# fhausmann/deepgrp

Hardware: AMD Instinct MI355X
Metric: Mbp/sec predicted (whole node) at window=200 stride=50, 5-class (higher is better)
Workload: dtype f16

## Files before the change

### deepgrp_amd/csrc/gru_shared.h

```cpp
#pragma once
#include "dgrp_model.h"

typedef _Float16 half8 __attribute__((ext_vector_type(8)));
typedef float f32x16 __attribute__((ext_vector_type(16)));
typedef float f32x4 __attribute__((ext_vector_type(4)));
typedef _Float16 half4 __attribute__((ext_vector_type(4)));

#define DGRP_WG_WINDOWS 16

struct gru_rec {
    int64_t idx_off, n, out_row, nwin;
    dgrp_placement place;
    int64_t win_first;
    int64_t pad_;
};

struct gru_params {
    const uint8_t *idx;
    int64_t n, s, w0, nw;
    dgrp_placement place;
    const uint4 *pack;
    const float *ffb;
    float *out;
    void *avg;
    int avg_f32;
    int T, C, nfrag, mode;
    int Tp;
    int ospan;
    const struct gru_rec *recs;
    const int64_t *wg_first;
    int64_t nrec;
    int64_t avgw;
    const uint4 *pack_lo;
    int lo_tile_off;
    float zfold;
    const uint4 *pack16;
    const float *xtab;
    int xtab_off;
    const uint4 *stream;
    const uint4 *packw;
    const float *xtabw;
    int avg_up;
};

__device__ __forceinline__ float sigmoid_from_scaled(float a) { return __builtin_amdgcn_rcpf(1.0f + __builtin_amdgcn_exp2f(a)); }
__device__ __forceinline__ float tanh_from_scaled(float a) { return 1.0f - 2.0f * __builtin_amdgcn_rcpf(1.0f + __builtin_amdgcn_exp2f(a)); }
typedef float f32x2 __attribute__((ext_vector_type(2)));
__device__ __forceinline__ f32x2 rcp1p_exp2_pair(float a0, float a1)
{
    f32x2 e = { __builtin_amdgcn_exp2f(a0), __builtin_amdgcn_exp2f(a1) };
    e = e + 1.0f;
    return f32x2{ __builtin_amdgcn_rcpf(e.x), __builtin_amdgcn_rcpf(e.y) };
}
__device__ __forceinline__ float fast_tanh(float x) { return tanh_from_scaled(2.8853900817779268f * x); }

template <int N>
__device__ __forceinline__ float row_ror(float x)
{
    return __builtin_bit_cast(float, __builtin_amdgcn_update_dpp(0, __builtin_bit_cast(int, x), 0x120 | N, 0xf, 0xf, false));
}
template <int N>
__device__ __forceinline__ float row_max_ror(float x)
{
    float r;
    asm("s_nop 1\n\tv_max_f32_dpp %0, %1, %1 row_ror:%2 row_mask:0xf bank_mask:0xf" : "=v"(r) : "v"(x), "n"(N));
    return r;
}
template <int CTRL>
__device__ __forceinline__ float quad_perm(float x)
{
    return __builtin_bit_cast(float, __builtin_amdgcn_update_dpp(0, __builtin_bit_cast(int, x), CTRL, 0xf, 0xf, false));
}
__device__ __forceinline__ float row_allmax(float x)
{
    return row_max_ror<1>(row_max_ror<2>(row_max_ror<4>(row_max_ror<8>(x))));
}
__device__ __forceinline__ float row_allsum(float x)
{
    x += row_ror<8>(x); x += row_ror<4>(x); x += row_ror<2>(x); return x + row_ror<1>(x);
}

typedef __attribute__((address_space(3))) unsigned lds_u32;
typedef __attribute__((address_space(1))) unsigned glb_u32;
__device__ __forceinline__ void lds_atomic_max(unsigned *p, unsigned v)
{
    (void)__hip_atomic_fetch_max((lds_u32 *)p, v, __ATOMIC_RELAXED, __HIP_MEMORY_SCOPE_WORKGROUP);
}
__device__ __forceinline__ void global_atomic_max(unsigned *p, unsigned v)
{
    (void)__hip_atomic_fetch_max((glb_u32 *)p, v, __ATOMIC_RELAXED, __HIP_MEMORY_SCOPE_AGENT);
}

__host__ __device__ static inline int gru_lds_hbuf(int UP, int pad = 8) { return 2 * 32 * (UP + pad) * 2; }
__host__ __device__ static inline int gru_lds_dpart(int NW) { return 2 * NW * 64 * 16; }
__host__ __device__ static inline int gru_lds_seq(int Tp) { return DGRP_WG_WINDOWS * Tp; }
__host__ __device__ static inline int gru_lds_meta() { return DGRP_WG_WINDOWS * 8 + DGRP_WG_WINDOWS * 4; }

struct wg_ctx {
    _Float16 *hbuf;
    float *dpart;
    uint8_t *seqs;
    int64_t *row0s;
    int *rowoff;
    unsigned *obuf;
    int64_t wg_w, lo;
    int nvalid;
};

template <int MODE>
__device__ __forceinline__ int64_t wg_record_at(const gru_params &pin, gru_params &p, int64_t g)
{
    if (MODE == 1 || !pin.recs) return g;
    int64_t lo_r = 0, hi_r = pin.nrec;
    while (hi_r - lo_r > 1) {
        const int64_t mid = (lo_r + hi_r) >> 1;
        if (pin.wg_first[mid] <= g) lo_r = mid; else hi_r = mid;
    }
    const gru_rec rc = pin.recs[lo_r];
    p.idx = pin.idx + rc.idx_off;
    p.n = rc.n;
    if (MODE == 0) p.out = pin.out + rc.out_row * pin.C;
    p.place = rc.place;
    p.w0 = 0;
    p.nw = rc.nwin;
    p.avgw = rc.win_first;
    return g - pin.wg_first[lo_r];
}
template <int MODE>
__device__ __forceinline__ int64_t wg_record(const gru_params &pin, gru_params &p) { return wg_record_at<MODE>(pin, p, blockIdx.x); }

template <int NW, int MODE, int HPAD = 8>
__device__ __forceinline__ wg_ctx wg_setup(const gru_params &p, unsigned char *smem, int64_t bid)
{
    constexpr int UP = 32 * NW, HS = UP + HPAD;
    wg_ctx c;
    c.hbuf = reinterpret_cast<_Float16 *>(smem);
    c.dpart = reinterpret_cast<float *>(smem + gru_lds_hbuf(UP, HPAD));
    c.seqs = smem + gru_lds_hbuf(UP, HPAD) + gru_lds_dpart(NW);
    c.row0s = reinterpret_cast<int64_t *>(c.seqs + gru_lds_seq(p.Tp));
    c.rowoff = reinterpret_cast<int *>(c.row0s + DGRP_WG_WINDOWS);
    c.obuf = reinterpret_cast<unsigned *>(c.rowoff + DGRP_WG_WINDOWS);
    const int tid = threadIdx.x, T = p.T, C = p.C;
    c.wg_w = p.w0 + bid * DGRP_WG_WINDOWS;
    c.nvalid = (int)min((int64_t)DGRP_WG_WINDOWS, p.w0 + p.nw - c.wg_w);
    for (int i = tid; i < DGRP_WG_WINDOWS * T; i += 64 * NW) {
        const int wi = i / T, t = i - wi * T;
        c.seqs[wi * p.Tp + t] = wi < c.nvalid ? p.idx[(c.wg_w + wi) * p.s + t] : (uint8_t)4;
    }
    for (int i = tid; i < 32 * HS; i += 64 * NW) c.hbuf[i] = (_Float16)0.0f;
    c.lo = 0;
    if (MODE == 0) {
        const int64_t a = dgrp_place_row(p.place, c.wg_w, p.s), b = dgrp_place_row(p.place, c.wg_w + c.nvalid - 1, p.s);
        c.lo = a < b ? a : b;
        for (int i = tid; i < p.ospan * C; i += 64 * NW) c.obuf[i] = 0u;
    }
    if (tid < DGRP_WG_WINDOWS) {
        int64_t r0 = -1;
        int off = -1;
        if (tid < c.nvalid) {
            r0 = MODE == 0 ? dgrp_place_row(p.place, c.wg_w + tid, p.s) : (c.wg_w + tid - p.w0 + p.avgw) * (int64_t)T;
            if (MODE == 0 && r0 >= c.lo && r0 - c.lo + T <= p.ospan) off = (int)(r0 - c.lo);
        }
        c.row0s[tid] = r0;
        c.rowoff[tid] = off;
    }
    __syncthreads();
    return c;
}

template <int MODE>
__device__ __forceinline__ void emit_value(const gru_params &p, const wg_ctx &c, int off, int64_t row0, int t, int cls, float val)
{
    if (MODE == 0) {
        if (off >= 0) {
            lds_atomic_max(c.obuf + (off + t) * p.C + cls, __float_as_uint(val));
        } else {
            const int64_t row = row0 + t;
            if (row < p.n) global_atomic_max(reinterpret_cast<unsigned *>(p.out) + row * p.C + cls, __float_as_uint(val));
        }
    } else {
        p.out[(row0 + t) * p.C + cls] = val;
    }
}

template <int NW, int MODE>
__device__ __forceinline__ void finish_register(const gru_params &p, const wg_ctx &c, int t, int reg, float fbias, int off, int64_t row0)
{
    const int lane = threadIdx.x & 63, cls = lane & 15;
    const float *dp = c.dpart + ((size_t)(t & 1) * 4 + reg) * NW * 64 + lane;
    float sum = dp[0];
#pragma unroll
    for (int w = 1; w < NW; ++w) sum += dp[w * 64];
    const int wi = 4 * (lane >> 4) + reg;
    const float lg = cls < p.C ? sum + fbias : -INFINITY;
    float val = lg;
    if (MODE != 2) {
        const float m = row_allmax(lg);
        const float e = __builtin_amdgcn_exp2f(1.4426950408889634f * (lg - m));
        val = e * __builtin_amdgcn_rcpf(row_allsum(e));
    }
    if (cls < p.C && wi < c.nvalid) emit_value<MODE>(p, c, off, row0, t, cls, val);
}

template <int NW>
__device__ __forceinline__ void flush_image(const gru_params &p, const wg_ctx &c)
{
    __syncthreads();
    unsigned *gout = reinterpret_cast<unsigned *>(p.out) + c.lo * p.C;
    const int64_t lim = (p.n - c.lo) * p.C;
    for (int i = threadIdx.x; i < p.ospan * p.C; i += 64 * NW) {
        const unsigned v = c.obuf[i];
        if (v != 0u && i < lim) global_atomic_max(gout + i, v);
    }
}

__device__ __forceinline__ void split_avg_store_lane(const gru_params &p, int64_t wg_w, int tt, int UP, int wave, int lane, half8 a0, half8 a1,
                                                     half8 l0, half8 l1)
{
    const int64_t at = ((wg_w + (lane & 15) - p.w0 + p.avgw) * (int64_t)p.T + tt) * UP + 32 * wave + 8 * (lane >> 4);
    if (p.avg_f32) {
        float *dst = reinterpret_cast<float *>(p.avg) + at;
        typedef unsigned u32x4_ __attribute__((ext_vector_type(4)));
        const _Float16 hf = (_Float16)0.5f;
        const u32x4_ A0 = __builtin_bit_cast(u32x4_, a0), A1 = __builtin_bit_cast(u32x4_, a1);
        const u32x4_ L0 = __builtin_bit_cast(u32x4_, l0 * hf), L1 = __builtin_bit_cast(u32x4_, l1 * hf);
        float v[8];
#pragma unroll
        for (int k = 0; k < 4; ++k) {
            float f0, f1, r0, r1;
            asm("v_fma_mix_f32 %0, %1, 0.5, %2 op_sel_hi:[1,0,1]" : "=v"(f0) : "v"(A0[k]), "v"(L0[k]));
            asm("v_fma_mix_f32 %0, %1, 0.5, %2 op_sel:[1,0,1] op_sel_hi:[1,0,1]" : "=v"(f1) : "v"(A0[k]), "v"(L0[k]));
            asm("v_fma_mix_f32 %0, %1, 0.5, %2 op_sel_hi:[1,0,1]" : "=v"(r0) : "v"(A1[k]), "v"(L1[k]));
            asm("v_fma_mix_f32 %0, %1, 0.5, %2 op_sel:[1,0,1] op_sel_hi:[1,0,1]" : "=v"(r1) : "v"(A1[k]), "v"(L1[k]));
            v[2 * k] = f0 + r0;
            v[2 * k + 1] = f1 + r1;
        }
        *reinterpret_cast<f32x4 *>(dst) = f32x4{ v[0], v[1], v[2], v[3] };
        *reinterpret_cast<f32x4 *>(dst + 4) = f32x4{ v[4], v[5], v[6], v[7] };
        return;
    }
    const _Float16 hf = (_Float16)0.5f;
    const half8 av = (a0 * hf + a1 * hf) + (l0 + l1) * hf;
    *reinterpret_cast<half8 *>(reinterpret_cast<_Float16 *>(p.avg) + at) = av;
}
__device__ __forceinline__ void split_avg_store(const gru_params &p, int64_t wg_w, int tt, int UP, int wave, half8 a0, half8 a1,
                                                half8 l0, half8 l1)
{
    split_avg_store_lane(p, wg_w, tt, UP, wave, threadIdx.x & 63, a0, a1, l0, l1);
}

struct split_gate_tmp { float er, e2, g, A, zt, d, n; };
template <bool ONERCP, int OP>
__device__ __forceinline__ void split_gate_op(split_gate_tmp &t, float ar, float ag, float az, float ax, float &s)
{
#pragma clang fp contract(off)
    if constexpr (OP == 0) t.er = __builtin_amdgcn_exp2f(ar);
    else if constexpr (OP == 1) t.e2 = __builtin_amdgcn_exp2f(az);
    else if constexpr (OP == 2) t.er = t.er + 1.0f;
    else if constexpr (OP == 3) t.er = __builtin_amdgcn_rcpf(t.er);
    else if constexpr (OP == 4) t.g = __builtin_fmaf(t.er, ag, ax);
    else if constexpr (OP == 5) t.A = __builtin_amdgcn_exp2f(t.g);
    else if constexpr (OP == 6) t.A = t.A + 1.0f;
    else if constexpr (ONERCP) {
        if constexpr (OP == 7) t.zt = __builtin_fmaf(0.5f, t.e2, 1.0f);
        else if constexpr (OP == 8) t.d = t.A * t.zt;
        else if constexpr (OP == 9) t.n = __builtin_fmaf(s, t.A, -t.e2);
        else if constexpr (OP == 10) t.d = __builtin_amdgcn_rcpf(t.d);
        else s = t.n * t.d;
    } else {
        if constexpr (OP == 7) t.zt = t.e2 + 1.0f;
        else if constexpr (OP == 8) t.d = __builtin_amdgcn_rcpf(t.A);
        else if constexpr (OP == 9) t.n = __builtin_fmaf(-2.0f, t.d, 1.0f);
        else if constexpr (OP == 10) t.zt = __builtin_amdgcn_rcpf(t.zt);
        else { const float df = s - t.n; s = __builtin_fmaf(t.zt, df, t.n); }
    }
}
#define DGRP_SPLIT_GATE_OPS 12
template <bool ONERCP>
__device__ __forceinline__ float split_gate_chain(float ar, float ag, float az, float ax, float s)
{
    split_gate_tmp t;
    split_gate_op<ONERCP, 0>(t, ar, ag, az, ax, s); split_gate_op<ONERCP, 1>(t, ar, ag, az, ax, s);
    split_gate_op<ONERCP, 2>(t, ar, ag, az, ax, s); split_gate_op<ONERCP, 3>(t, ar, ag, az, ax, s);
    split_gate_op<ONERCP, 4>(t, ar, ag, az, ax, s); split_gate_op<ONERCP, 5>(t, ar, ag, az, ax, s);
    split_gate_op<ONERCP, 6>(t, ar, ag, az, ax, s); split_gate_op<ONERCP, 7>(t, ar, ag, az, ax, s);
    split_gate_op<ONERCP, 8>(t, ar, ag, az, ax, s); split_gate_op<ONERCP, 9>(t, ar, ag, az, ax, s);
    split_gate_op<ONERCP, 10>(t, ar, ag, az, ax, s); split_gate_op<ONERCP, 11>(t, ar, ag, az, ax, s);
    return s;
}
template <bool ONERCP> __device__ __forceinline__ float split_state_h(float s)
{
#pragma clang fp contract(off)
    return ONERCP ? s + 1.0f : s;
}
__device__ __forceinline__ uint2 split_pack4(const float h[4])
{
    uint2 r;
    asm("v_cvt_pk_f16_f32 %0, %1, %2" : "=v"(r.x) : "v"(h[0]), "v"(h[1]));
    asm("v_cvt_pk_f16_f32 %0, %1, %2" : "=v"(r.y) : "v"(h[2]), "v"(h[3]));
    return r;
}
__device__ __forceinline__ void split_residual4(float h[4], uint2 hi)
{
    asm("v_fma_mix_f32 %0, %1, -1.0, %0 op_sel_hi:[1,0,0]" : "+v"(h[0]) : "v"(hi.x));
    asm("v_fma_mix_f32 %0, %1, -1.0, %0 op_sel:[1,0,0] op_sel_hi:[1,0,0]" : "+v"(h[1]) : "v"(hi.x));
    asm("v_fma_mix_f32 %0, %1, -1.0, %0 op_sel_hi:[1,0,0]" : "+v"(h[2]) : "v"(hi.y));
    asm("v_fma_mix_f32 %0, %1, -1.0, %0 op_sel:[1,0,0] op_sel_hi:[1,0,0]" : "+v"(h[3]) : "v"(hi.y));
}
__device__ __forceinline__ void split_hi_lo4(const float h[4], uint2 &hv, uint2 &lv)
{
    float r[4] = { h[0], h[1], h[2], h[3] };
    hv = split_pack4(r);
    split_residual4(r, hv);
    lv = split_pack4(r);
}

__device__ __forceinline__ float wave_half_sum(float h, float half)
{
#pragma clang fp contract(off)
    float t = half * h;
    asm("s_nop 1\n\tv_fmac_f32_dpp %0, %1, %2 row_ror:8 row_mask:0xf bank_mask:0xf" : "+v"(t) : "v"(h), "v"(half));
    return t;
}

__device__ __forceinline__ void split_lstm_cell(float ai, float af, float ac, float ao, float &c, float &h)
{
#pragma clang fp contract(off)
    const float ig = __builtin_amdgcn_rcpf(1.0f + __builtin_amdgcn_exp2f(ai));
    const float fg = __builtin_amdgcn_rcpf(1.0f + __builtin_amdgcn_exp2f(af));
    const float tc = __builtin_fmaf(-2.0f, __builtin_amdgcn_rcpf(1.0f + __builtin_amdgcn_exp2f(ac)), 1.0f);
    const float it = ig * tc;
    c = __builtin_fmaf(fg, c, it);
    const float og = __builtin_amdgcn_rcpf(1.0f + __builtin_amdgcn_exp2f(ao));
    const float e2 = __builtin_amdgcn_exp2f(2.8853900817779268f * c);
    const float th = __builtin_fmaf(-2.0f, __builtin_amdgcn_rcpf(1.0f + e2), 1.0f);
    h = og * th;
}
```

### deepgrp_amd/csrc/gru_split2.hip

```cpp
#include "gru_shared.h"
#include <mutex>
#include <type_traits>

typedef unsigned u32x4 __attribute__((ext_vector_type(4)));

namespace {

constexpr int NW = 4, UP = 128, KS = 4, HPAD = 16, HS = UP + HPAD;
constexpr int XT_PITCH = 4 * 128 * 4 + 32;

struct split2_weights {
    u32x4 hi[3][KS][2], lo[3][KS][2];
    u32x4 Bd_hi, Bd_lo;
};

#define LOAD2(a, pa, b, pb)                                                                                             \
    asm volatile("global_load_dwordx4 %0, %2, off\n\tglobal_load_dwordx4 %1, %3, off\n\ts_waitcnt vmcnt(0)"            \
                 : "=&a"(a), "=&a"(b) : "v"(pa), "v"(pb) : "memory")

#define MFMA_R(acc, Wf, b) asm volatile("v_mfma_f32_16x16x32_f16 %0, %1, %2, %0" : "+v"(acc) : "a"(Wf), "v"(b))
#define MFMA_D(acc, a, Wf) asm volatile("v_mfma_f32_16x16x32_f16 %0, %1, %2, %0" : "+v"(acc) : "v"(a), "a"(Wf))
#define MFMA_DZ(acc, a, Wf) asm volatile("v_mfma_f32_16x16x32_f16 %0, %1, %2, 0" : "=&v"(acc) : "v"(a), "a"(Wf))

struct tile_state {
    gru_params p;
    wg_ctx ctx;
    unsigned hcur, hnxt, lcur, lnxt;
    unsigned myseq;
    float h[16];
    f32x4 ar[4], ag[4], az[4], ax[4];
    f32x4 dpl;
    unsigned tabf, tabr;
    half8 f0h[2], f0l[2];
    int p_off;
    int64_t p_row0;
    bool pr_on;
};

template <int MODE, bool ONERCP>
__global__ void __launch_bounds__(256) __attribute__((amdgpu_waves_per_eu(1, 1))) gru_split2_kernel(const gru_params pin, int half_bytes)
{
    extern __shared__ __attribute__((aligned(16))) unsigned char smem[];
    const int tid = threadIdx.x;
    const int lane = tid & 63;
    const int wave = __builtin_amdgcn_readfirstlane(tid >> 6);
    const int T = pin.T, C = pin.C;

    split2_weights W;
    {
        const uint4 *p16 = pin.pack16 + (size_t)wave * 48 * 64 + lane;
#pragma unroll
        for (int g = 0; g < 3; ++g)
#pragma unroll
            for (int ks = 0; ks < KS; ++ks) {
                LOAD2(W.hi[g][ks][0], p16 + (size_t)(g * 8 + ks * 2) * 64, W.hi[g][ks][1], p16 + (size_t)(g * 8 + ks * 2 + 1) * 64);
                LOAD2(W.lo[g][ks][0], p16 + (size_t)(24 + g * 8 + ks * 2) * 64, W.lo[g][ks][1], p16 + (size_t)(24 + g * 8 + ks * 2 + 1) * 64);
            }
        const uint4 *mypack = pin.pack + (size_t)wave * pin.nfrag * 64 + lane;
        LOAD2(W.Bd_hi, mypack + (size_t)(3 * (2 * KS + 1) + 1) * 64, W.Bd_lo, mypack + (size_t)(3 * (2 * KS + 1) + 2) * 64);
    }
    for (int i = tid; i < 5 * 512; i += 256)
        *reinterpret_cast<float *>(smem + pin.xtab_off + (i / 512) * XT_PITCH + (i % 512) * 4) = pin.xtab[i];

    const int wi = lane & 15, q4 = lane >> 4;
    const int cls = lane & 15;
    const float fbias = cls < C ? pin.ffb[cls] : 0.0f;
    const int pwi = 4 * (lane >> 4) + wave;
    const unsigned frag_lane = (unsigned)(wi * HS + 8 * q4) * 2;
    const unsigned dense_lane = (unsigned)(wi * HS + 32 * wave + 8 * q4) * 2;
    const unsigned pub_lane = (unsigned)(wi * HS + 32 * wave + 4 * q4) * 2;
    const unsigned tab_lane = (unsigned)pin.xtab_off + (unsigned)(32 * wave + 4 * q4) * 4;

    tile_state S0, S1;
    auto setup = [&](tile_state &Z, int x) {
        unsigned char *base = smem + (size_t)x * half_bytes;
        _Float16 *lbuf = reinterpret_cast<_Float16 *>(base + pin.lo_tile_off);
        for (int i = tid; i < 32 * HS; i += 256) lbuf[i] = (_Float16)0.0f;
        Z.p = pin;
        const int64_t bid = wg_record_at<MODE>(pin, Z.p, 2 * (int64_t)blockIdx.x + x);
        Z.ctx = wg_setup<NW, MODE, HPAD>(Z.p, base, bid);
        Z.hcur = (unsigned)x * half_bytes;
        Z.hnxt = Z.hcur + 32 * HS * 2;
        Z.lcur = (unsigned)x * half_bytes + pin.lo_tile_off;
        Z.lnxt = Z.lcur + 32 * HS * 2;
        Z.myseq = (unsigned)(Z.ctx.seqs - smem) + wi * pin.Tp;
#pragma unroll
        for (int i = 0; i < 16; ++i) Z.h[i] = ONERCP ? -1.0f : 0.0f;
        Z.p_off = Z.ctx.rowoff[pwi];
        Z.p_row0 = Z.ctx.row0s[pwi];
        Z.pr_on = cls < C && pwi < Z.ctx.nvalid;
    };
    setup(S0, 0);
    setup(S1, 1);

    auto lds16 = [&](unsigned off) -> half8 { return *reinterpret_cast<const half8 *>(smem + off); };
    auto ldsf4 = [&](unsigned off) -> f32x4 { return *reinterpret_cast<const f32x4 *>(smem + off); };
    auto tab_rows = [&](tile_state &Z, uint32_t bf, uint32_t br) {
        bf = bf < 4 ? bf : 4;
        br = br < 4 ? 3 - br : 4;
        Z.tabf = tab_lane + bf * XT_PITCH;
        Z.tabr = tab_lane + br * XT_PITCH;
    };
    auto acc_init = [&](tile_state &Z, int g, int sub) {
        const f32x4 v = ldsf4(((sub & 1) ? Z.tabr : Z.tabf) + g * 512 + (sub >> 1) * 64);
        if (g == 0) Z.ar[sub] = v; else if (g == 1) Z.ag[sub] = v; else Z.az[sub] = v;
    };

    struct frag_ring { half8 h[2][2], l[2][2]; };
    struct dense_ops { half8 a0, a1, l0, l1; };
    struct fin_state { float d[NW], lg, m, e, s; };
    auto phase = [&](auto do_x, auto do_y, auto do_f, tile_state &X, tile_state &Y, int tx, int ty) __attribute__((always_inline)) {
        constexpr bool DO_X = decltype(do_x)::value, DO_Y = decltype(do_y)::value, DO_F = decltype(do_f)::value;
        frag_ring F;
        dense_ops D;
        fin_state fs;
        split_gate_tmp gt[16];
        float pbh[4][4];
        uint2 pbhv[4], pblv[4];
        uint32_t xp_bf = 4, xp_br = 4;
        const int td = ty - 1;
        const int tf = tx - 2;
        if constexpr (DO_X) { F.h[0][0] = X.f0h[0]; F.h[0][1] = X.f0h[1]; F.l[0][0] = X.f0l[0]; F.l[0][1] = X.f0l[1]; }
#define GAP __builtin_amdgcn_sched_barrier(0);
#define M_K(ks, n)                                                                                               \
    if constexpr (DO_X) {                                                                                        \
        constexpr int ps_ = (n) / 12, g_ = ((n) % 12) / 4, uh_ = ((n) % 4) / 2, rh_ = (n) % 2, sub_ = 2 * uh_ + rh_; \
        const half8 &b_ = ps_ == 1 ? F.l[(ks) & 1][rh_] : F.h[(ks) & 1][rh_];                                    \
        const u32x4 &w_ = ps_ == 2 ? W.lo[g_][ks][uh_] : W.hi[g_][ks][uh_];                                      \
        if constexpr (g_ == 0) MFMA_R(X.ar[sub_], w_, b_);                                                       \
        else if constexpr (g_ == 1) MFMA_R(X.ag[sub_], w_, b_);                                                  \
        else MFMA_R(X.az[sub_], w_, b_);                                                                         \
    }
#define M_D(i)                                                                                                   \
    if constexpr (DO_X) {                                                                                        \
        if constexpr ((i) == 0) MFMA_DZ(X.dpl, D.a0, W.Bd_hi);                                                   \
        else if constexpr ((i) == 1) MFMA_D(X.dpl, D.a1, W.Bd_hi);                                               \
        else if constexpr ((i) == 2) MFMA_D(X.dpl, D.a0, W.Bd_lo);                                               \
        else if constexpr ((i) == 3) MFMA_D(X.dpl, D.a1, W.Bd_lo);                                               \
        else if constexpr ((i) == 4) MFMA_D(X.dpl, D.l0, W.Bd_hi);                                               \
        else MFMA_D(X.dpl, D.l1, W.Bd_hi);                                                                       \
    }
#define PF(ks)                                                                                                   \
    if constexpr (DO_X) {                                                                                        \
        F.h[(ks) & 1][0] = lds16(X.hcur + frag_lane + 64 * (ks)); F.h[(ks) & 1][1] = lds16(X.hcur + frag_lane + 16 * HS * 2 + 64 * (ks)); \
        F.l[(ks) & 1][0] = lds16(X.lcur + frag_lane + 64 * (ks)); F.l[(ks) & 1][1] = lds16(X.lcur + frag_lane + 16 * HS * 2 + 64 * (ks)); \
    }
#define RDD                                                                                                      \
    if constexpr (DO_X) {                                                                                        \
        D.a0 = lds16(X.hcur + dense_lane); D.a1 = lds16(X.hcur + dense_lane + 16 * HS * 2);                      \
        D.l0 = lds16(X.lcur + dense_lane); D.l1 = lds16(X.lcur + dense_lane + 16 * HS * 2);                      \
        if (MODE == 2 && tx > 0 && (lane & 15) < X.ctx.nvalid)                                                   \
            split_avg_store(X.p, X.ctx.wg_w, tx - 1, UP, wave, D.a0, D.a1, D.l0, D.l1);                          \
    }
#define AXL(sub) \
    if constexpr (DO_Y) Y.ax[sub] = ldsf4((((sub) & 1) ? Y.tabr : Y.tabf) + 3 * 512 + ((sub) >> 1) * 64);
#define DS(i)                                                                                                    \
    if constexpr (DO_Y) Y.ctx.dpart[((size_t)(td & 1) * 4 * NW + wave) * 64 + lane + (i) * NW * 64] = Y.dpl[i];
#define G(e, op) \
    if constexpr (DO_Y) split_gate_op<ONERCP, op>(gt[e], Y.ar[(e) / 4][(e) % 4], Y.ag[(e) / 4][(e) % 4], Y.az[(e) / 4][(e) % 4], Y.ax[(e) / 4][(e) % 4], Y.h[e]);
#define PB(g, op)                                                                                                \
    if constexpr (DO_Y) {                                                                                        \
        if constexpr ((op) == 0) {                                                                               \
            pbh[g][0] = split_state_h<ONERCP>(Y.h[4 * (g)]); pbh[g][1] = split_state_h<ONERCP>(Y.h[4 * (g) + 1]); \
            pbh[g][2] = split_state_h<ONERCP>(Y.h[4 * (g) + 2]); pbh[g][3] = split_state_h<ONERCP>(Y.h[4 * (g) + 3]); \
        } else if constexpr ((op) == 1) {                                                                        \
            pbhv[g] = split_pack4(pbh[g]);                                                                       \
        } else if constexpr ((op) == 2) {                                                                        \
            split_residual4(pbh[g], pbhv[g]);                                                                    \
        } else if constexpr ((op) == 3) {                                                                        \
            pblv[g] = split_pack4(pbh[g]);                                                                       \
        } else {                                                                                                 \
            *reinterpret_cast<uint2 *>(smem + Y.hnxt + pub_lane + ((g) & 1) * 16 * HS * 2 + ((g) >> 1) * 32) = pbhv[g]; \
            *reinterpret_cast<uint2 *>(smem + Y.lnxt + pub_lane + ((g) & 1) * 16 * HS * 2 + ((g) >> 1) * 32) = pblv[g]; \
        }                                                                                                        \
    }
#define BAR                                                                                                      \
    if constexpr (DO_Y) {                                                                                        \
        asm volatile("s_waitcnt lgkmcnt(0)\n\ts_barrier" ::: "memory");                                          \
        unsigned sw_ = Y.hcur; Y.hcur = Y.hnxt; Y.hnxt = sw_;                                                    \
        sw_ = Y.lcur; Y.lcur = Y.lnxt; Y.lnxt = sw_;                                                             \
    }
#define RD0                                                                                                      \
    if constexpr (DO_Y) {                                                                                        \
        Y.f0h[0] = lds16(Y.hcur + frag_lane); Y.f0h[1] = lds16(Y.hcur + frag_lane + 16 * HS * 2);                \
        Y.f0l[0] = lds16(Y.lcur + frag_lane); Y.f0l[1] = lds16(Y.lcur + frag_lane + 16 * HS * 2);                \
    }
#define XP(op)                                                                                                   \
    if constexpr (DO_Y) {                                                                                        \
        if constexpr ((op) == 0) { xp_bf = smem[Y.myseq + ty + 1]; xp_br = smem[Y.myseq + T - 2 - ty]; }                       \
        else tab_rows(Y, xp_bf, xp_br);                                                                          \
    }
#define CI(g, sub) \
    if constexpr (DO_Y) acc_init(Y, g, sub);
#define FN(op)                                                                                                   \
    if constexpr (DO_F) {                                                                                        \
        if constexpr ((op) == 0) {                                                                               \
            const float *dp_ = X.ctx.dpart + ((size_t)(tf & 1) * 4 + wave) * NW * 64 + lane;                     \
            fs.d[0] = dp_[0]; fs.d[1] = dp_[64]; fs.d[2] = dp_[128]; fs.d[3] = dp_[192];                         \
        } else if constexpr ((op) == 1) {                                                                        \
            const float sum_ = ((fs.d[0] + fs.d[1]) + fs.d[2]) + fs.d[3];                                        \
            fs.lg = cls < C ? sum_ + fbias : -INFINITY;                                                          \
        } else if constexpr ((op) == 2) { if (MODE != 2) fs.m = row_max_ror<8>(fs.lg); }                         \
        else if constexpr ((op) == 3) { if (MODE != 2) fs.m = row_max_ror<4>(fs.m); }                            \
        else if constexpr ((op) == 4) { if (MODE != 2) fs.m = row_max_ror<2>(fs.m); }                            \
        else if constexpr ((op) == 5) { if (MODE != 2) fs.m = row_max_ror<1>(fs.m); }                            \
        else if constexpr ((op) == 6) { if (MODE != 2) fs.e = __builtin_amdgcn_exp2f(1.4426950408889634f * (fs.lg - fs.m)); } \
        else if constexpr ((op) == 7) { if (MODE != 2) fs.s = fs.e + row_ror<8>(fs.e); }                         \
        else if constexpr ((op) == 8) { if (MODE != 2) fs.s += row_ror<4>(fs.s); }                               \
        else if constexpr ((op) == 9) { if (MODE != 2) fs.s += row_ror<2>(fs.s); }                               \
        else if constexpr ((op) == 10) { if (MODE != 2) fs.s += row_ror<1>(fs.s); }                              \
        else if constexpr ((op) == 11) { if (MODE != 2) fs.e *= __builtin_amdgcn_rcpf(fs.s); }                   \
        else { if (X.pr_on && tf >= 0) emit_value<MODE>(X.p, X.ctx, X.p_off, X.p_row0, tf, cls, MODE == 2 ? fs.lg : fs.e); } \
    }
#include "gru_split2_phase.inc"
#undef GAP
#undef M_K
#undef M_D
#undef PF
#undef RDD
#undef AXL
#undef DS
#undef G
#undef PB
#undef BAR
#undef RD0
#undef XP
#undef CI
#undef FN
    };
    const std::true_type yes;
    const std::false_type no;

    auto first_step = [&](tile_state &Z) {
        tab_rows(Z, smem[Z.myseq], smem[Z.myseq + T - 1]);
#pragma unroll
        for (int g = 0; g < 3; ++g)
#pragma unroll
            for (int sub = 0; sub < 4; ++sub) acc_init(Z, g, sub);
        Z.f0h[0] = lds16(Z.hcur + frag_lane); Z.f0h[1] = lds16(Z.hcur + frag_lane + 16 * HS * 2);
        Z.f0l[0] = lds16(Z.lcur + frag_lane); Z.f0l[1] = lds16(Z.lcur + frag_lane + 16 * HS * 2);
    };
    first_step(S0);
    first_step(S1);
    phase(yes, no, no, S0, S1, 0, 0);
#define EDGE_PAD do { asm volatile("s_nop 15\n\ts_nop 7"); __builtin_amdgcn_sched_barrier(0); } while (0)
    EDGE_PAD;
    for (int t = 0; t + 1 < T; ++t) {
        phase(yes, yes, yes, S1, S0, t, t);
        phase(yes, yes, yes, S0, S1, t + 1, t);
        EDGE_PAD;
    }
    phase(yes, yes, yes, S1, S0, T - 1, T - 1);
    phase(no, yes, yes, S0, S1, T, T - 1);

    auto drain = [&](tile_state &Z, bool prev_open) {
        const half8 a0 = lds16(Z.hcur + dense_lane), a1 = lds16(Z.hcur + dense_lane + 16 * HS * 2);
        const half8 l0 = lds16(Z.lcur + dense_lane), l1 = lds16(Z.lcur + dense_lane + 16 * HS * 2);
        if (MODE == 2 && (lane & 15) < Z.ctx.nvalid) split_avg_store(Z.p, Z.ctx.wg_w, T - 1, UP, wave, a0, a1, l0, l1);
        f32x4 d;
        MFMA_DZ(d, a0, W.Bd_hi); MFMA_D(d, a1, W.Bd_hi); MFMA_D(d, a0, W.Bd_lo); MFMA_D(d, a1, W.Bd_lo); MFMA_D(d, l0, W.Bd_hi); MFMA_D(d, l1, W.Bd_hi);
        asm volatile("s_nop 15\n\ts_nop 7" : "+v"(d));
        float *dw = Z.ctx.dpart + ((size_t)((T - 1) & 1) * 4 * NW + wave) * 64 + lane;
#pragma unroll
        for (int reg = 0; reg < 4; ++reg) dw[reg * NW * 64] = d[reg];
        __syncthreads();
        if (prev_open && T > 1) finish_register<NW, MODE>(Z.p, Z.ctx, T - 2, wave, fbias, Z.p_off, Z.p_row0);
        finish_register<NW, MODE>(Z.p, Z.ctx, T - 1, wave, fbias, Z.p_off, Z.p_row0);
        if (MODE == 0 && pin.ospan > 0) flush_image<NW>(Z.p, Z.ctx);
    };
    drain(S0, false);
    drain(S1, true);
}

template <int MODE, bool ONERCP>
int launch_split2(const gru_params &p, int64_t groups, int half_bytes, hipStream_t stream)
{
    static std::once_flag configured;
    static hipError_t cfg_err = hipSuccess;
    std::call_once(configured, [] { cfg_err = hipFuncSetAttribute((const void *)gru_split2_kernel<MODE, ONERCP>, hipFuncAttributeMaxDynamicSharedMemorySize, 160 * 1024); });
    DGRP_HIP(cfg_err);
    hipLaunchKernelGGL((gru_split2_kernel<MODE, ONERCP>), dim3((unsigned)((groups + 1) / 2)), dim3(256), (size_t)2 * half_bytes + 5 * XT_PITCH, stream, p, half_bytes);
    DGRP_LAUNCH_CHECK();
    return DGRP_OK;
}

}

int dgrp_split2_launch(const gru_params &p, int64_t groups, int half_bytes, bool onercp, hipStream_t stream)
{
    if (onercp)
        return p.mode == 0 ? launch_split2<0, true>(p, groups, half_bytes, stream)
             : p.mode == 1 ? launch_split2<1, true>(p, groups, half_bytes, stream) : launch_split2<2, true>(p, groups, half_bytes, stream);
    return p.mode == 0 ? launch_split2<0, false>(p, groups, half_bytes, stream)
         : p.mode == 1 ? launch_split2<1, false>(p, groups, half_bytes, stream) : launch_split2<2, false>(p, groups, half_bytes, stream);
}
```

Baseline: 553.8.

## Load overlapping window span once and batch weight loads in split2 GRU prologue

Adds a setup variant that, when the overlapping 16-window span fits in LDS, copies the contiguous sequence span with aligned 16-byte loads and indexes windows by stride instead of copying each window's bytes separately. Weight loads no longer wait after every pair, so all global loads are issued before a single wait. The two tiles' setups now share one barrier instead of one each, and the low-tile zeroing uses 16-byte stores. This targets prologue latency and redundant global reads, at the cost of a fallback path and more complex indexing.

```diff
diff --git a/deepgrp_amd/csrc/gru_shared.h b/deepgrp_amd/csrc/gru_shared.h
--- a/deepgrp_amd/csrc/gru_shared.h
+++ b/deepgrp_amd/csrc/gru_shared.h
@@ -168,6 +168,67 @@
     return c;
 }
 
+template <int NW, int MODE, int HPAD>
+__device__ __forceinline__ wg_ctx wg_setup_span(const gru_params &p, unsigned char *smem, int64_t bid, unsigned &seq0, unsigned &pitch)
+{
+    constexpr int UP = 32 * NW, HS = UP + HPAD;
+    wg_ctx c;
+    c.hbuf = reinterpret_cast<_Float16 *>(smem);
+    c.dpart = reinterpret_cast<float *>(smem + gru_lds_hbuf(UP, HPAD));
+    c.seqs = smem + gru_lds_hbuf(UP, HPAD) + gru_lds_dpart(NW);
+    c.row0s = reinterpret_cast<int64_t *>(c.seqs + gru_lds_seq(p.Tp));
+    c.rowoff = reinterpret_cast<int *>(c.row0s + DGRP_WG_WINDOWS);
+    c.obuf = reinterpret_cast<unsigned *>(c.rowoff + DGRP_WG_WINDOWS);
+    const int tid = threadIdx.x, T = p.T, C = p.C;
+    c.wg_w = p.w0 + bid * DGRP_WG_WINDOWS;
+    c.nvalid = (int)min((int64_t)DGRP_WG_WINDOWS, p.w0 + p.nw - c.wg_w);
+    seq0 = 0;
+    pitch = (unsigned)p.Tp;
+    if ((DGRP_WG_WINDOWS - 1) * p.s + T + 15 <= (int64_t)gru_lds_seq(p.Tp)) {
+        pitch = (unsigned)p.s;
+        if (c.nvalid > 0) {
+            const uint8_t *src = p.idx + c.wg_w * p.s, *end = p.idx + p.n;
+            seq0 = (unsigned)(reinterpret_cast<uintptr_t>(src) & 15);
+            const uint8_t *a0 = src - seq0;
+            const int pieces = (int)((seq0 + (c.nvalid - 1) * p.s + T + 15) >> 4);
+            for (int i = tid; i < pieces; i += 64 * NW) {
+                const uint8_t *g = a0 + 16 * i;
+                if (g >= p.idx && g + 16 <= end) {
+                    *reinterpret_cast<uint4 *>(c.seqs + 16 * i) = *reinterpret_cast<const uint4 *>(g);
+                } else {
+                    for (int k = 0; k < 16; ++k) c.seqs[16 * i + k] = (g + k >= p.idx && g + k < end) ? g[k] : (uint8_t)4;
+                }
+            }
+        }
+    } else {
+        for (int i = tid; i < DGRP_WG_WINDOWS * T; i += 64 * NW) {
+            const int wi = i / T, t = i - wi * T;
+            c.seqs[wi * p.Tp + t] = wi < c.nvalid ? p.idx[(c.wg_w + wi) * p.s + t] : (uint8_t)4;
+        }
+    }
+    {
+        uint4 *h4 = reinterpret_cast<uint4 *>(c.hbuf);
+        for (int i = tid; i < 32 * HS * 2 / 16; i += 64 * NW) h4[i] = uint4{ 0u, 0u, 0u, 0u };
+    }
+    c.lo = 0;
+    if (MODE == 0) {
+        const int64_t a = dgrp_place_row(p.place, c.wg_w, p.s), b = dgrp_place_row(p.place, c.wg_w + c.nvalid - 1, p.s);
+        c.lo = a < b ? a : b;
+        for (int i = tid; i < p.ospan * C; i += 64 * NW) c.obuf[i] = 0u;
+    }
+    if (tid < DGRP_WG_WINDOWS) {
+        int64_t r0 = -1;
+        int off = -1;
+        if (tid < c.nvalid) {
+            r0 = MODE == 0 ? dgrp_place_row(p.place, c.wg_w + tid, p.s) : (c.wg_w + tid - p.w0 + p.avgw) * (int64_t)T;
+            if (MODE == 0 && r0 >= c.lo && r0 - c.lo + T <= p.ospan) off = (int)(r0 - c.lo);
+        }
+        c.row0s[tid] = r0;
+        c.rowoff[tid] = off;
+    }
+    return c;
+}
+
 template <int MODE>
 __device__ __forceinline__ void emit_value(const gru_params &p, const wg_ctx &c, int off, int64_t row0, int t, int cls, float val)
 {
diff --git a/deepgrp_amd/csrc/gru_split2.hip b/deepgrp_amd/csrc/gru_split2.hip
--- a/deepgrp_amd/csrc/gru_split2.hip
+++ b/deepgrp_amd/csrc/gru_split2.hip
@@ -15,8 +15,9 @@
 };
 
 #define LOAD2(a, pa, b, pb)                                                                                             \
-    asm volatile("global_load_dwordx4 %0, %2, off\n\tglobal_load_dwordx4 %1, %3, off\n\ts_waitcnt vmcnt(0)"            \
+    asm volatile("global_load_dwordx4 %0, %2, off\n\tglobal_load_dwordx4 %1, %3, off"                                    \
                  : "=&a"(a), "=&a"(b) : "v"(pa), "v"(pb) : "memory")
+#define LOAD_WAIT() asm volatile("s_waitcnt vmcnt(0)" ::: "memory")
 
 #define MFMA_R(acc, Wf, b) asm volatile("v_mfma_f32_16x16x32_f16 %0, %1, %2, %0" : "+v"(acc) : "a"(Wf), "v"(b))
 #define MFMA_D(acc, a, Wf) asm volatile("v_mfma_f32_16x16x32_f16 %0, %1, %2, %0" : "+v"(acc) : "v"(a), "a"(Wf))
@@ -58,6 +59,7 @@
             }
         const uint4 *mypack = pin.pack + (size_t)wave * pin.nfrag * 64 + lane;
         LOAD2(W.Bd_hi, mypack + (size_t)(3 * (2 * KS + 1) + 1) * 64, W.Bd_lo, mypack + (size_t)(3 * (2 * KS + 1) + 2) * 64);
+        LOAD_WAIT();
     }
     for (int i = tid; i < 5 * 512; i += 256)
         *reinterpret_cast<float *>(smem + pin.xtab_off + (i / 512) * XT_PITCH + (i % 512) * 4) = pin.xtab[i];
@@ -72,26 +74,27 @@
     const unsigned tab_lane = (unsigned)pin.xtab_off + (unsigned)(32 * wave + 4 * q4) * 4;
 
     tile_state S0, S1;
-    auto setup = [&](tile_state &Z, int x) {
+    auto stage = [&](tile_state &Z, int x) {
         unsigned char *base = smem + (size_t)x * half_bytes;
-        _Float16 *lbuf = reinterpret_cast<_Float16 *>(base + pin.lo_tile_off);
-        for (int i = tid; i < 32 * HS; i += 256) lbuf[i] = (_Float16)0.0f;
+        uint4 *lbuf = reinterpret_cast<uint4 *>(base + pin.lo_tile_off);
+        for (int i = tid; i < 32 * HS * 2 / 16; i += 256) lbuf[i] = uint4{ 0u, 0u, 0u, 0u };
         Z.p = pin;
         const int64_t bid = wg_record_at<MODE>(pin, Z.p, 2 * (int64_t)blockIdx.x + x);
-        Z.ctx = wg_setup<NW, MODE, HPAD>(Z.p, base, bid);
+        unsigned seq0, pitch;
+        Z.ctx = wg_setup_span<NW, MODE, HPAD>(Z.p, base, bid, seq0, pitch);
         Z.hcur = (unsigned)x * half_bytes;
         Z.hnxt = Z.hcur + 32 * HS * 2;
         Z.lcur = (unsigned)x * half_bytes + pin.lo_tile_off;
         Z.lnxt = Z.lcur + 32 * HS * 2;
-        Z.myseq = (unsigned)(Z.ctx.seqs - smem) + wi * pin.Tp;
+        Z.myseq = (unsigned)(Z.ctx.seqs - smem) + seq0 + wi * pitch;
 #pragma unroll
         for (int i = 0; i < 16; ++i) Z.h[i] = ONERCP ? -1.0f : 0.0f;
+    };
+    auto bind = [&](tile_state &Z) {
         Z.p_off = Z.ctx.rowoff[pwi];
         Z.p_row0 = Z.ctx.row0s[pwi];
         Z.pr_on = cls < C && pwi < Z.ctx.nvalid;
     };
-    setup(S0, 0);
-    setup(S1, 1);
 
     auto lds16 = [&](unsigned off) -> half8 { return *reinterpret_cast<const half8 *>(smem + off); };
     auto ldsf4 = [&](unsigned off) -> f32x4 { return *reinterpret_cast<const f32x4 *>(smem + off); };
@@ -240,10 +243,15 @@
         Z.f0h[0] = lds16(Z.hcur + frag_lane); Z.f0h[1] = lds16(Z.hcur + frag_lane + 16 * HS * 2);
         Z.f0l[0] = lds16(Z.lcur + frag_lane); Z.f0l[1] = lds16(Z.lcur + frag_lane + 16 * HS * 2);
     };
+#define EDGE_PAD do { asm volatile("s_nop 15\n\ts_nop 7"); __builtin_amdgcn_sched_barrier(0); } while (0)
+    stage(S0, 0);
+    stage(S1, 1);
+    __syncthreads();
+    bind(S0);
+    bind(S1);
     first_step(S0);
     first_step(S1);
     phase(yes, no, no, S0, S1, 0, 0);
-#define EDGE_PAD do { asm volatile("s_nop 15\n\ts_nop 7"); __builtin_amdgcn_sched_barrier(0); } while (0)
     EDGE_PAD;
     for (int t = 0; t + 1 < T; ++t) {
         phase(yes, yes, yes, S1, S0, t, t);
```

Result: no change. 556.2 (median of 6 runs) (+0.4%).
